# SuperbTUM/real-time-ReID-tracking

Hardware: AMD Instinct MI355X
Metric: crops/sec embedded + NxM distmat ms, ResNet18-SE 128x256 (higher is better)
Workload: dtype f16x3; 1 GPU; BASELINE configs[1]: ResNet18-SE embed 4096 distinct uint8 crops (128x256) per GPU + 4096x4096 L2 distmat; crops_per_gpu=4096, embed_dim=512, chunk=1024

## Files before the change

real-time-reid-tracking_amd/csrc/api.hip:

```cpp
#include "reid_internal.h"
#include <stdarg.h>
#include <stdio.h>
#include <string.h>
#include <stdlib.h>
#include <sstream>

static thread_local char g_err[1024] = "";

void reid_set_error(const char* fmt, ...) {
    va_list ap;
    va_start(ap, fmt);
    vsnprintf(g_err, sizeof(g_err), fmt, ap);
    va_end(ap);
}

extern "C" const char* reid_last_error(void) { return g_err; }

extern "C" int reid_device_count(int* n) {
    ARG_CHECK(n);
    HIP_TRY(hipGetDeviceCount(n));
    return REID_OK;
}

extern "C" int reid_ctx_create(int device, reid_ctx** out) {
// ... 7 lines not shown
    DeviceGuard _dev_guard(device);
    reid_ctx* c = new reid_ctx();
    c->device = device;
    if (const char* e = getenv("REID_SWIN_CHUNK_MAX")) {
        const int v = atoi(e);
        if (v > 0 && v < c->swin_chunk_cap) c->swin_chunk_cap = v;
    }
    if (const char* e = getenv("REID_KNN_WIDE_MIN")) c->knn_wide_min = atoll(e);
    HIP_TRY(hipStreamCreateWithFlags(&c->own_stream, hipStreamNonBlocking));
    c->stream = c->own_stream;
    HIP_TRY(hipHostMalloc((void**)&c->fault, 64, hipHostMallocMapped));
    memset(c->fault, 0, 64);
    HIP_TRY(hipEventCreate(&c->t0));
    HIP_TRY(hipEventCreate(&c->t1));
    *out = c;
    return REID_OK;
}

extern "C" int reid_ctx_destroy(reid_ctx* ctx) {
    if (!ctx) return REID_OK;
    DeviceGuard _dev_guard(ctx->device);
    hipStreamSynchronize(ctx->stream);
    comm_release(ctx);
    swin_release(ctx);
    for (int i = 0; i < 2; ++i)
        if (ctx->frame_ev[i]) hipEventDestroy(ctx->frame_ev[i]);
    if (ctx->copy_ev) hipEventDestroy(ctx->copy_ev);
    for (hipEvent_t e : ctx->pipe_ev) hipEventDestroy(e);
    for (int i = 0; i < 2; ++i) {
        if (ctx->fwd_ev[i]) hipEventDestroy(ctx->fwd_ev[i]);
        if (ctx->match_ev[i]) hipEventDestroy(ctx->match_ev[i]);
    }
    if (ctx->join_ev) hipEventDestroy(ctx->join_ev);
    if (ctx->match_stream) { hipStreamSynchronize(ctx->match_stream); hipStreamDestroy(ctx->match_stream); }
    if (ctx->copy_stream) { hipStreamSynchronize(ctx->copy_stream); hipStreamDestroy(ctx->copy_stream); }
    for (auto& kv : ctx->ws) hipFree(kv.second.first);
    for (auto& kv : ctx->split_w) hipFree(kv.second);
    for (auto& kv : ctx->pinned) hipHostFree(kv.second.first);
    if (ctx->se18.blob) hipFree(ctx->se18.blob);
    if (ctx->se18.blob16) hipFree(ctx->se18.blob16);
    if (ctx->se18.stem_w16) hipFree(ctx->se18.stem_w16);
    if (ctx->se18.stem_w16s) hipFree(ctx->se18.stem_w16s);
    for (int i = 0; i < 2; ++i)
        if (ctx->se18.l1_conv2_w16s[i]) hipFree(ctx->se18.l1_conv2_w16s[i]);
    if (ctx->se18.zero_page) hipFree(ctx->se18.zero_page);
    if (ctx->se18.ep) hipFree(ctx->se18.ep);
    for (auto& e : ctx->ev_pool) { hipEventDestroy(e.first); hipEventDestroy(e.second); }
    for (auto& p : ctx->pending) { hipEventDestroy(p.a); hipEventDestroy(p.b); }
    hipEventDestroy(ctx->t0);
    hipEventDestroy(ctx->t1);
    hipStreamDestroy(ctx->own_stream);
    if (ctx->fault) hipHostFree(ctx->fault);
    delete ctx;
    return REID_OK;
}

extern "C" int reid_ctx_set_stream(reid_ctx* ctx, void* s) {
    ARG_CHECK(ctx);
    CTX_GUARD(ctx);
    ctx->stream = s ? (hipStream_t)s : ctx->own_stream;
    return REID_OK;
}

extern "C" int reid_ctx_set_null_stream(reid_ctx* ctx) {
    ARG_CHECK(ctx);
    CTX_GUARD(ctx);
// ... 105 lines not shown
        reid_set_error("%s: side indices are pending (reid_ctx_set_side_index) but the loaded weights carry no table for them", what);
        ctx->side_idx.clear();
        return REID_ERR_STATE;
    }
    if (ctx->side_cursor + (size_t)n > ctx->side_idx.size()) {
        reid_set_error("%s: %d images but only %zu side indices are pending", what, n, ctx->side_idx.size() - ctx->side_cursor);
        ctx->side_idx.clear();
        return REID_ERR_ARG;
    }
    const int32_t* h = ctx->side_idx.data() + ctx->side_cursor;
    for (int i = 0; i < n; ++i)
        if (h[i] >= rows) {
            reid_set_error("%s: side index %d of image %d is outside the table of %d rows", what, h[i], i, rows);
            ctx->side_idx.clear();
            return REID_ERR_ARG;
        }
    int32_t* d;
    REID_TRY(ctx_ws(ctx, "side.idx", (size_t)n * 4, (void**)&d));
    HIP_TRY(hipMemcpyAsync(d, h, (size_t)n * 4, hipMemcpyHostToDevice, ctx->stream));
    HIP_TRY(hipStreamSynchronize(ctx->stream));
    ctx->side_cursor += n;
    if (ctx->side_cursor == ctx->side_idx.size()) ctx->side_idx.clear();
    *d_idx = d;
    return REID_OK;
}

extern "C" int reid_ctx_set_debug_keep(reid_ctx* ctx, int on) {
    ARG_CHECK(ctx);
    CTX_GUARD(ctx);
    ctx->debug_keep = on < 0 ? 0 : (on > 2 ? 2 : on);
    return REID_OK;
}

int ctx_ws(reid_ctx* ctx, const char* name, size_t bytes, void** out) {
    auto it = ctx->ws.find(name);
    if (it != ctx->ws.end() && it->second.second >= bytes) {
        *out = it->second.first;
        return REID_OK;
    }
    bool regrow = false;
    if (it != ctx->ws.end()) {
        HIP_TRY(hipStreamSynchronize(ctx->stream));
        HIP_TRY(hipFree(it->second.first));
        ctx->ws.erase(it);
        regrow = true;
    }
    void* p = nullptr;
    size_t cap = bytes < 256 ? 256 : bytes;
    if (regrow) cap += cap / 2 < ((size_t)1 << 30) ? cap / 2 : ((size_t)1 << 30);
    hipError_t e = hipMalloc(&p, cap);
    if (e != hipSuccess) {
        reid_set_error("hipMalloc(%zu) for workspace '%s' failed: %s", cap, name, hipGetErrorString(e));
        return REID_ERR_NOMEM;
    }
    ctx->ws[name] = {p, cap};
    *out = p;
    return REID_OK;
}

int ctx_pinned(reid_ctx* ctx, const char* name, size_t bytes, void** out) {
    auto it = ctx->pinned.find(name);
    if (it != ctx->pinned.end() && it->second.second >= bytes) {
        *out = it->second.first;
        return REID_OK;
    }
    if (it != ctx->pinned.end()) {
        HIP_TRY(hipStreamSynchronize(ctx->stream));
// ... 596 lines not shown
        REID_TRY(launch_norm_finalize(ctx, b.stats, n, tiles, k.c, half, hw, k.in_gamma, k.in_beta, k.bn1_scale, k.bn1_shift,
                                      b.a_scale, b.a_shift));
        REID_TRY(conv_gemm(ctx, A_IM2COL, c1, n, Ho, Wo, k.c, k.conv2_w, k.c, 3, 3, 1, 1, 9 * k.c, b.a_scale, b.a_shift, 1,
                           k.bn2_scale, k.bn2_shift, k.ds ? nullptr : cur, k.ds ? 0 : 1, b.stats, y));
        }
        const float* shortcut = cur;
        if (k.ds) {
            REID_TRY(conv_gemm(ctx, A_IM2COL, cur, n, H, W, k.cin, k.ds_w, k.c, 1, 1, k.stride, 0, k.cin, nullptr, nullptr, 0,
                               k.ds_scale, k.ds_shift, nullptr, 0, nullptr, sc, 0, cur16));
            shortcut = sc;
        }
        float* out = c1;
        if (w.arch == 1) {
            REID_TRY(launch_ta_tail(ctx, y, shortcut, n, Ho, Wo, k.c, k.ta, out));
        } else if (w.arch == 2) {
            REID_TRY(launch_ema_tail(ctx, y, shortcut, n, Ho, Wo, k.c, k.ema, out));
        } else if (ctx->f32_conv == 1) {
            bool fp32_read = true;
            if (cur16 && !keep && i < 7 && w.blk[i + 1].ds && ctx->pack_epilogue) {
                const Se18Block& nx = w.blk[i + 1];
                fp32_read = !(conv_split_path(ctx, n, Ho, Wo, nx.cin, nx.c, 3, 3, nx.stride, 1) &&
                              conv_split_path(ctx, n, Ho, Wo, nx.cin, nx.c, 1, 1, nx.stride, 0));
            }
            REID_TRY(launch_se_tail(ctx, b.stats, n, tiles, k.c, k.mid, hw, k.se_w1, k.se_w2, y, shortcut, fp32_read ? out : nullptr,
                                    i < 7 ? cur16 : nullptr));
        } else {
            REID_TRY(launch_se_finalize(ctx, b.stats, n, tiles, k.c, k.mid, hw, k.se_w1, k.se_w2, b.se));
            REID_TRY(launch_se_combine(ctx, y, shortcut, b.se, n, hw, k.c, out));
        }
        b.stage[2 + i] = out;
        cur = out;
        H = Ho;
        W = Wo;
    }
    REID_TRY(launch_gem_neck(ctx, cur, n, H * W, 512, w.gem_p, w.neck_scale, w.neck_shift, b.gem, d_emb));
    {
        const int32_t* d_cam;
        REID_TRY(ctx_take_side(ctx, n, w.num_cams, "reid_embed (camera bias)", &d_cam));
        if (d_cam) REID_TRY(launch_add_indexed_rows(ctx, d_emb, n, 1, 512, w.cam_bias, d_cam, w.cam_factor));
    }
    b.stage[10] = b.gem;
    if (d_logits) {
        if (!w.cls_w) {
            reid_set_error("logits requested but the weight blob has no classifier (cls.w)");
            return REID_ERR_STATE;
        }
        GemmParams p;
        memset(&p, 0, sizeof(p));
        p.A = d_emb; p.lda = 512;
        p.B = w.cls_w; p.ldb = 512;
        p.M = n; p.N = w.num_class; p.K = 512;
        p.C = d_logits; p.ldc = w.num_class;
        REID_TRY(launch_gemm_f32(ctx, A_DENSE, E_BIAS, p, REID_K_CONV_GEMM, 2.0 * n * w.num_class * 512,
                                 ((double)n * 512 + (double)w.num_class * 512 + (double)n * w.num_class) * 4.0));
    }
    ctx->last_n = n;
    ctx->last_f16 = false;
    for (int s = 0; s < 11; ++s) ctx->stage_ptr[s] = b.stage[s];
    return REID_OK;
}

int conv_gemm16(reid_ctx* ctx, int amode, const _Float16* x, int n, int H, int W, int Cin, const _Float16* wgt, int Cout,
                       int R, int S, int stride, int pad, int K, const float* col_scale, const float* col_shift,
                       const _Float16* residual, int relu, float* stats, _Float16* out, int Hp, int Wp) {
    Gemm16Params p;
    memset(&p, 0, sizeof(p));
// ... 160 lines not shown

extern "C" int reid_debug_stage(reid_ctx* ctx, int stage, float* out, size_t max_floats, size_t* count) {
    ARG_CHECK(ctx && stage >= 0 && stage < 11 && out);
    CTX_GUARD(ctx);
    if (!ctx->debug_keep || ctx->last_n <= 0) {
        reid_set_error("reid_debug_stage: enable reid_ctx_set_debug_keep before the embed call");
        return REID_ERR_STATE;
    }
    const size_t total = kStageElems[stage] * (size_t)ctx->last_n;
    if (count) *count = total;
    const size_t ncopy = total < max_floats ? total : max_floats;
    if (ctx->last_f16 && stage < 10) {
        std::vector<_Float16> tmp(ncopy);
        HIP_TRY(hipMemcpyAsync(tmp.data(), ctx->stage_ptr[stage], ncopy * 2, hipMemcpyDeviceToHost, ctx->stream));
        HIP_TRY(hipStreamSynchronize(ctx->stream));
        for (size_t i = 0; i < ncopy; ++i) out[i] = (float)tmp[i];
        return REID_OK;
    }
    HIP_TRY(hipMemcpyAsync(out, ctx->stage_ptr[stage], ncopy * 4, hipMemcpyDeviceToHost, ctx->stream));
    HIP_TRY(hipStreamSynchronize(ctx->stream));
    return REID_OK;
}

int ctx_pipe_events(reid_ctx* ctx, int passes) {
    if (!ctx->copy_stream) HIP_TRY(hipStreamCreateWithFlags(&ctx->copy_stream, hipStreamNonBlocking));
    while ((int)ctx->pipe_ev.size() < 2 * passes) {
        hipEvent_t e;
        HIP_TRY(hipEventCreateWithFlags(&e, hipEventDisableTiming));
        ctx->pipe_ev.push_back(e);
    }
    return REID_OK;
}

extern "C" int reid_embed_u8_dev(reid_ctx* ctx, const uint8_t* d_crops, int n, float* d_emb, float* d_logits) {
    ARG_CHECK(ctx && d_crops && d_emb && n >= 0);
    CTX_ENTER(ctx);
    const int nc = ctx->se18.num_class;
    for (int i = 0; i < n; i += ctx->chunk) {
        const int m = n - i < ctx->chunk ? n - i : ctx->chunk;
        REID_TRY(seres18_run(ctx, d_crops + (size_t)i * IMG_H * IMG_W * 3, true, m, d_emb + (size_t)i * 512,
                                 d_logits ? d_logits + (size_t)i * nc : nullptr));
    }
    return REID_OK;
}

extern "C" int reid_embed_u8(reid_ctx* ctx, const uint8_t* crops, int n, float* emb, float* logits) {
    ARG_CHECK(ctx && crops && emb && n >= 0);
    CTX_ENTER(ctx);
    if (n == 0) return REID_OK;
    const int nc = ctx->se18.num_class;
    uint8_t* d_in;
    float *d_emb, *d_log = nullptr;
    const size_t crop_b = (size_t)IMG_H * IMG_W * 3;
    REID_TRY(ctx_ws(ctx, "io.in", (size_t)n * crop_b, (void**)&d_in));
    REID_TRY(ctx_ws(ctx, "io.emb", (size_t)n * 512 * 4, (void**)&d_emb));
    if (logits) REID_TRY(ctx_ws(ctx, "io.logits", (size_t)n * nc * 4 + 16, (void**)&d_log));
    REID_TRY(host_passes(
        ctx, n, ctx->chunk,
        [&](int i, int m, hipStream_t s) -> int {
            HIP_TRY(hipMemcpyAsync(d_in + (size_t)i * crop_b, crops + (size_t)i * crop_b, (size_t)m * crop_b, hipMemcpyHostToDevice, s));
            return REID_OK;
        },
        [&](int i, int m) -> int {
            return seres18_run(ctx, d_in + (size_t)i * crop_b, true, m, d_emb + (size_t)i * 512, d_log ? d_log + (size_t)i * nc : nullptr);
        },
        [&](int i, int m, hipStream_t s) -> int {
            HIP_TRY(hipMemcpyAsync(emb + (size_t)i * 512, d_emb + (size_t)i * 512, (size_t)m * 512 * 4, hipMemcpyDeviceToHost, s));
            if (logits) HIP_TRY(hipMemcpyAsync(logits + (size_t)i * nc, d_log + (size_t)i * nc, (size_t)m * nc * 4, hipMemcpyDeviceToHost, s));
            return REID_OK;
        }));
    return ctx_fault_status(ctx);
}

extern "C" int reid_embed_f32_nchw_dev(reid_ctx* ctx, const float* d_x, int n, float* d_emb, float* d_logits) {
    ARG_CHECK(ctx && d_x && d_emb && n >= 0);
    CTX_ENTER(ctx);
    const int nc = ctx->se18.num_class;
    const size_t img = (size_t)IMG_H * IMG_W * 3;
    for (int i = 0; i < n; i += ctx->chunk) {
        const int m = n - i < ctx->chunk ? n - i : ctx->chunk;
        float* nhwc;
        REID_TRY(ctx_ws(ctx, "se18.in_nhwc", (size_t)m * img * 4, (void**)&nhwc));
        REID_TRY(launch_nchw_to_nhwc3(ctx, d_x + (size_t)i * img, m, IMG_H, IMG_W, nhwc));
        REID_TRY(seres18_run(ctx, nhwc, false, m, d_emb + (size_t)i * 512, d_logits ? d_logits + (size_t)i * nc : nullptr));
    }
    return REID_OK;
}

extern "C" int reid_embed_f32_nchw(reid_ctx* ctx, const float* x, int n, float* emb, float* logits) {
    ARG_CHECK(ctx && x && emb && n >= 0);
    CTX_ENTER(ctx);
    if (n == 0) return REID_OK;
    const int nc = ctx->se18.num_class;
    const size_t img = (size_t)IMG_H * IMG_W * 3;
    float *d_in, *d_emb, *d_log = nullptr;
    REID_TRY(ctx_ws(ctx, "io.in", (size_t)n * img * 4, (void**)&d_in));
    REID_TRY(ctx_ws(ctx, "io.emb", (size_t)n * 512 * 4, (void**)&d_emb));
    if (logits) REID_TRY(ctx_ws(ctx, "io.logits", (size_t)n * nc * 4 + 16, (void**)&d_log));
    REID_TRY(host_passes(
        ctx, n, ctx->chunk,
        [&](int i, int m, hipStream_t s) -> int {
            HIP_TRY(hipMemcpyAsync(d_in + (size_t)i * img, x + (size_t)i * img, (size_t)m * img * 4, hipMemcpyHostToDevice, s));
            return REID_OK;
        },
        [&](int i, int m) -> int {
            float* nhwc;
            REID_TRY(ctx_ws(ctx, "se18.in_nhwc", (size_t)m * img * 4, (void**)&nhwc));
            REID_TRY(launch_nchw_to_nhwc3(ctx, d_in + (size_t)i * img, m, IMG_H, IMG_W, nhwc));
            return seres18_run(ctx, nhwc, false, m, d_emb + (size_t)i * 512, d_log ? d_log + (size_t)i * nc : nullptr);
        },
        [&](int i, int m, hipStream_t s) -> int {
            HIP_TRY(hipMemcpyAsync(emb + (size_t)i * 512, d_emb + (size_t)i * 512, (size_t)m * 512 * 4, hipMemcpyDeviceToHost, s));
            if (logits) HIP_TRY(hipMemcpyAsync(logits + (size_t)i * nc, d_log + (size_t)i * nc, (size_t)m * nc * 4, hipMemcpyDeviceToHost, s));
            return REID_OK;
        }));
    return ctx_fault_status(ctx);
}

int embed_ragged_enqueue(reid_ctx* ctx, const char* tag, const uint8_t* packed, const int64_t* offsets, const int32_t* hw, int n,
// ... 519 lines not shown
```

real-time-reid-tracking_amd/csrc/conv3x3_f16.hip:

```cpp
#include "reid_internal.h"
#include "conv3x3_geom.h"
#include <type_traits>

typedef _Float16 f16;
typedef f16 half8 __attribute__((ext_vector_type(8)));
typedef float f32x16 __attribute__((ext_vector_type(16)));

namespace {

#define GPTR(p) ((const __attribute__((address_space(1))) void*)(p))
#define LPTR(p) ((__attribute__((address_space(3))) void*)(uintptr_t)(p))
#define WAIT_VMCNT(n) asm volatile("s_waitcnt vmcnt(%0)" ::"n"(n) : "memory")
#define RAW_BARRIER() asm volatile("s_barrier" ::: "memory")

template <int TW, int IMGS, int BN, int LW, bool SPLIT = false, bool PAIR = false>
__global__ __launch_bounds__(LW ? 768 : 512) void conv3x3_f16_kernel(const Gemm16Params p) {
    static_assert(!PAIR || (SPLIT && LW == 1 && BN == 128), "PAIR: fp32-class build, loader waves, 128-wide tiles");
    constexpr int TH = 256 / (IMGS * TW);
    constexpr int WP = TW + 2, HP = TH + 2;
    constexpr int NPX = IMGS * HP * WP;
    constexpr int NPI = (NPX + 7) / 8;
    constexpr int HPW = (NPI + 7) / 8;
    constexpr int HALO_BYTES = NPI * 1024;
    constexpr int B_BYTES = BN * 128;
// ... 699 lines not shown
        for (int a = 0; a < TM; ++a)
#pragma unroll
            for (int e = 0; e < 16; ++e) tile[c_row_natural<TW, IMGS>(wm, a, e, lh) * BN + lcol] = (f16)acc[a][b][e];
    }
    ESTAMP(te3);
    __syncthreads();
    constexpr int C8 = BN / 8;
    for (int idx = tid; idx < 256 * C8; idx += NTHR) {
        const int row = idx / C8, c8 = idx - row * C8;
        if (row < m_valid) *(half8*)(Cb + (long long)row * ldc + c8 * 8) = *(const half8*)(tile + row * BN + c8 * 8);
    }
    if (LW && p.diag && lane == 0 && blockIdx.x < 64) {
        asm volatile("s_waitcnt vmcnt(0)" ::: "memory");
        ESTAMP(te4);
        if (wave == 0) {
            unsigned long long* d2 = p.diag + 64 * 8 * 4 + blockIdx.x * 8;
            d2[0] = te1 - t_loop_end; d2[1] = te2 - te1; d2[2] = te3 - te2; d2[3] = te4 - te3;
        }
    }
}

template <int TW, int IMGS, int LW, bool SPLIT = false>
int launch_geom(reid_ctx* ctx, const Gemm16Params& p0) {
    Gemm16Params p = p0;
    p.fault = ctx->fault;
    p.general_epi = !ctx->split_lean_epi;
    p.pair_early = ctx->split_pair == 2;
    p.loader_prio = ctx->f16_loader_prio == 2 || (ctx->f16_loader_prio == 1 && SPLIT);
    p.frag_ahead = ctx->f16_frag_ahead;
    const int nmt = (p.M + 255) / 256;
    const int threads = LW ? 768 : 512;
    const int nchunk = p.Cin / 64;
    auto splitk = [&](int tiles, int bn, int sk) -> int {
        if (sk > 1) {
            float* ws;
            int* cnt;
            bool fresh = ctx->ws.find("conv16.splitk_cnt") == ctx->ws.end();
            REID_TRY(ctx_ws(ctx, "conv16.splitk_ws", (size_t)tiles * sk * 256 * bn * sizeof(float), (void**)&ws));
            REID_TRY(ctx_ws(ctx, "conv16.splitk_cnt", 256 * sizeof(int), (void**)&cnt));
            if (fresh) HIP_TRY(hipMemsetAsync(cnt, 0, 256 * sizeof(int), ctx->stream));
            p.split_k = sk; p.splitk_ws = ws; p.splitk_cnt = cnt;
        }
        return REID_OK;
    };
    const int tiles128 = p.N % 128 == 0 ? nmt * (p.N / 128) : 0;
#ifdef REID_EXPERIMENTS
    constexpr bool CAN_PAIR = SPLIT && LW == 1;
#else
    constexpr bool CAN_PAIR = false;
#endif
    const bool pair = CAN_PAIR && ctx->split_pair && p.split_terms == 3;
    if (tiles128 > 128) {
        if constexpr (CAN_PAIR) {
            if (pair) hipLaunchKernelGGL((conv3x3_f16_kernel<TW, IMGS, 128, LW, SPLIT, true>), dim3(tiles128), dim3(threads), 0, ctx->stream, p);
        }
        if (!pair) hipLaunchKernelGGL((conv3x3_f16_kernel<TW, IMGS, 128, LW, SPLIT>), dim3(tiles128), dim3(threads), 0, ctx->stream, p);
    } else {
        const int tiles64 = nmt * (p.N / 64);
        int best_bn = 64, best_sk = 1;
        double best = 1e30;
        auto consider = [&](int bn, int tiles, int sk, double bias) {
            if (tiles <= 0 || nchunk % sk != 0 || (sk > 1 && (!ctx->f16_split_k || tiles * sk > 256))) return;
            const double cost = (double)((tiles * sk + 255) / 256) * (nchunk / sk) * 9 * (bn == 128 ? 1.3 : 0.65) + (sk > 1 ? 2.0 : 0.0) + bias;
            if (cost < best) { best = cost; best_bn = bn; best_sk = sk; }
        };
        if (ctx->f16_wide_splitk && nchunk >= 16 && tiles128 >= 48) consider(128, tiles128, 4, -0.003);
// ... 137 lines not shown
```

real-time-reid-tracking_amd/csrc/conv3x3_x3.hip:

```cpp
#include "reid_internal.h"
#include "conv3x3_geom.h"
#include "lin_math.h"
#include <type_traits>
#include <utility>

typedef _Float16 f16;
typedef f16 half8 __attribute__((ext_vector_type(8)));
typedef float f32x16 __attribute__((ext_vector_type(16)));

namespace {

#define GPTR(p) ((const __attribute__((address_space(1))) void*)(p))
#define LPTR(p) ((__attribute__((address_space(3))) void*)(uintptr_t)(p))
#define RAW_BARRIER() asm volatile("s_barrier" ::: "memory")
#define LDS_READ(dst, addr, off) asm volatile("ds_read_b128 %0, %1 offset:%2" : "=v"(dst) : "v"(addr), "n"(off))

template <int N>
__device__ __forceinline__ void lgkm_wait2(half8& x, half8& y) { asm volatile("s_waitcnt lgkmcnt(%2)" : "+v"(x), "+v"(y) : "n"(N)); }
template <int N>
__device__ __forceinline__ void lgkm_wait1(half8& x) { asm volatile("s_waitcnt lgkmcnt(%1)" : "+v"(x) : "n"(N)); }

__device__ __forceinline__ void wait_vm(int n) {
    switch (n) {
        case 0: asm volatile("s_waitcnt vmcnt(0)" ::: "memory"); break;
// ... 1675 lines not shown
    while (ctx->f16_split_k && tiles * sk * 2 <= slots && ncr % (sk * 2) == 0 && sk * 2 <= (wide ? 8 : 4)) sk *= 2;
    const int cap = ctx->x3_sk_cap > 0 ? ctx->x3_sk_cap : 4;
    return sk > cap ? cap : sk;
}

static bool x3_wide_tiles(const reid_ctx* ctx, const Gemm16Params& p) {
    if (p.N % 128 != 0 || (p.W == 16 && (ctx->x3_narrow & 1)) || (p.W == 8 && (ctx->x3_narrow & 2))) return false;
    if (p.W == 8 && p.N == 256 && !(ctx->x3_narrow & 4)) {
        const int nmt = (p.M + 255) / 256, ncr = p.Cin / 3 / 32;
        const int t128 = nmt * 2, t64 = nmt * 4;
        const int s128 = x3_split(ctx, t128, ncr, true);
        (void)t64;
        if (t128 * s128 < 256) return false;
    }
    if (p.W == 8 && p.N == 512 && ctx->x3_l4_narrow_nmt > 0) {
        const int nmt = (p.M + 255) / 256, ncr = p.Cin / 3 / 32;
        const int t128 = nmt * 4, s128 = x3_split(ctx, t128, ncr, true);
        if (s128 == 4 && t128 * s128 > 256 && nmt <= ctx->x3_l4_narrow_nmt) return false;
        if (s128 == 1 && t128 % 256 != 0 && t128 % 256 <= 128) return false;
        if (s128 == 2 && t128 > 128 && t128 * 4 <= 768) return false;
    }
    return true;
}

static int x3_slots(const Gemm16Params& p, bool wide) { return (!wide && p.W == 8 && p.N == 512 && (p.M + 255) / 256 > 32) ? 768 : 512; }

template <int TW, int IMGS>
int launch_x3m16(reid_ctx* ctx, const Gemm16Params& p0) {
    Gemm16Params p = p0;
    const int nmt = (p.M + 255) / 256;
    const bool wide = x3_wide_tiles(ctx, p);
    const int tiles = nmt * (wide ? p.N / 128 : p.N / 64);
    const int sk = x3_split(ctx, tiles, p.Cin / 3 / 32, wide, x3_slots(p, wide));
    if (sk > 1) {
        float* ws;
        int* cnt;
        const bool fresh = ctx->ws.find("x3.splitk_cnt") == ctx->ws.end();
        ARG_CHECK(tiles <= 512);
        REID_TRY(ctx_ws(ctx, "x3.splitk_ws", (size_t)tiles * sk * 256 * (wide ? 128 : 64) * sizeof(float), (void**)&ws));
        REID_TRY(ctx_ws(ctx, "x3.splitk_cnt", 1024 * sizeof(int), (void**)&cnt));
        if (fresh) HIP_TRY(hipMemsetAsync(cnt, 0, 1024 * sizeof(int), ctx->stream));
        p.split_k = sk; p.splitk_ws = ws; p.splitk_cnt = cnt;
    } else {
        p.split_k = 1;
    }
    const bool unrolled = ctx->x3_unroll && (long long)p.M * (p.Cin / 3) * 4 < 0x7f000000ll && (long long)p.N * p.ldb * 2 < 0x7f000000ll;
    if (wide && unrolled) hipLaunchKernelGGL((conv3x3_x3u_kernel<TW, IMGS, 128, 2>), dim3(tiles * sk), dim3(256), 0, ctx->stream, p);
    else if (wide) hipLaunchKernelGGL((conv3x3_x3m16_kernel<TW, IMGS, 128>), dim3(tiles * sk), dim3(256), 0, ctx->stream, p);
    else if (unrolled && ctx->x3_unroll == 3) hipLaunchKernelGGL((conv3x3_x3u_kernel<TW, IMGS, 64, 3>), dim3(tiles * sk), dim3(256), 0, ctx->stream, p);
#ifdef REID_EXPERIMENTS
    else if (unrolled && ctx->x3_unroll == 4) hipLaunchKernelGGL((conv3x3_x3u_kernel<TW, IMGS, 64, 4>), dim3(tiles * sk), dim3(256), 0, ctx->stream, p);
    else if (unrolled && ctx->x3_unroll == 5) hipLaunchKernelGGL((conv3x3_x3u_kernel<TW, IMGS, 64, 3, 3>), dim3(tiles * sk), dim3(256), 0, ctx->stream, p);
#endif
    else hipLaunchKernelGGL((conv3x3_x3m16_kernel<TW, IMGS, 64>), dim3(tiles * sk), dim3(256), 0, ctx->stream, p);
    return REID_OK;
}

template <int TW, int IMGS>
void launch_x3(reid_ctx* ctx, const Gemm16Params& p) {
    const int nmt = (p.M + 255) / 256;
    if (p.N % 128 == 0) hipLaunchKernelGGL((conv3x3_x3_kernel<TW, IMGS, 128>), dim3(nmt * (p.N / 128)), dim3(256), 0, ctx->stream, p);
    else hipLaunchKernelGGL((conv3x3_x3_kernel<TW, IMGS, 64>), dim3(nmt * (p.N / 64)), dim3(256), 0, ctx->stream, p);
}

}

static int launch_tiles(const reid_ctx* ctx, const Gemm16Params& p) {
    const int nmt = (p.M + 255) / 256;
    return nmt * (x3_wide_tiles(ctx, p) ? p.N / 128 : p.N / 64);
}

bool conv3x3_x3_supported(const reid_ctx* ctx, const Gemm16Params& p) {
    if (!ctx->split_x3 || p.split_terms != 3 || p.Cin % 96 != 0 || p.N % 64 != 0 || p.M % 128 != 0 || !conv3x3_f16_supported(p)) return false;
    if (p.relu_from % 16 != 0 || (p.pack16 && p.pack_from % 32 != 0)) return false;
    if (p.N % 128 != 0 && ctx->split_x3 < 3) return false;
    const int nmt = (p.M + 255) / 256;
    const long long blocks = (long long)nmt * (p.N % 128 == 0 ? p.N / 128 : p.N / 64);
    if (blocks >= ctx->split_x3_min_blocks) return true;
    if (ctx->split_x3 < 2 || !ctx->split_x3_small) return false;
    if (ctx->split_x3_small == 1) return true;
    const int tiles = launch_tiles(ctx, p);
    if (p.W == 8) return true;
    if (p.W == 32) return p.M / 256 > 256 || tiles >= 384;
    return p.M / 256 > 128 || tiles >= 384;
}

int launch_conv3x3_x3(reid_ctx* ctx, const Gemm16Params& p0) {
    Gemm16Params p = p0;
    p.fault = ctx->fault;
    p.ablate |= ctx->x3_ablate;
    if (ctx->split_x3 >= 2) {
        if (p.W == 32) REID_TRY((launch_x3m16<32, 1>(ctx, p)));
        else if (p.W == 16) REID_TRY((launch_x3m16<16, 1>(ctx, p)));
        else REID_TRY((launch_x3m16<8, 2>(ctx, p)));
    } else if (p.W == 32) launch_x3<32, 1>(ctx, p);
    else if (p.W == 16) launch_x3<16, 1>(ctx, p);
    else launch_x3<8, 2>(ctx, p);
    LAUNCH_CHECK();
    return REID_OK;
}

#ifdef REID_EXPERIMENTS
int launch_chain(reid_ctx* ctx, const ChainParams& cp, int W) {
    ARG_CHECK(cp.n_img >= 1 && cp.n_img <= 64 && cp.n_stages >= 1 && cp.n_stages <= 8 && cp.counters && W == 8);
    const int blocks = cp.total_items < 512 ? cp.total_items : 512;
    hipLaunchKernelGGL((chain_kernel<8, 2, 128>), dim3(blocks), dim3(256), 0, ctx->stream, cp);
    LAUNCH_CHECK();
    return REID_OK;
}
#endif

bool conv_x3s_supported(const reid_ctx* ctx, const Gemm16Params& p) {
    if (!ctx->conv_x3s || ctx->split_x3 < 2 || p.split_terms != 3 || p.Cin % 96 != 0 || p.N % 128 != 0 || p.M % 128 != 0) return false;
    if (!((p.R == 1 || p.R == 3) && p.S == p.R && p.pad == (p.R - 1) / 2 && (p.stride == 1 || p.stride == 2))) return false;
    if (p.R == 3 && p.stride == 1) return false;
    if (p.relu_from % 16 != 0 || (p.pack16 && p.pack_from % 32 != 0)) return false;
    const long long a_bytes = (long long)(p.M / (p.Ho * p.Wo)) * p.H * p.W * (p.Cin / 3) * 4;
    return a_bytes < 0x7f000000ll && 128ll * p.ldb * 2 < 0x7f000000ll && 256ll * p.ldc * 4 < 0x7f000000ll && (long long)p.M * 2 < 0x7f000000ll;
}

int launch_conv_x3s(reid_ctx* ctx, const Gemm16Params& p0, int kind, double flops, double bytes) {
    Gemm16Params p = p0;
    p.fault = ctx->fault;
    p.ablate = 0;
    const int tiles = ((p.M + 255) / 256) * (p.N / 128), nq = p.R * p.S * (p.Cin / 3 / 32);
    int sk = 1;
    while (ctx->f16_split_k && tiles * sk * 2 <= 512 && nq / (sk * 2) >= 2 && sk * 2 <= ctx->x3s_sk_cap) sk *= 2;
    if (sk > 1) {
        float* ws;
        int* cnt;
        const bool fresh = ctx->ws.find("x3.splitk_cnt") == ctx->ws.end();
        ARG_CHECK(tiles <= 512);
        REID_TRY(ctx_ws(ctx, "x3.splitk_ws", (size_t)tiles * sk * 256 * 128 * sizeof(float), (void**)&ws));
        REID_TRY(ctx_ws(ctx, "x3.splitk_cnt", 1024 * sizeof(int), (void**)&cnt));
        if (fresh) HIP_TRY(hipMemsetAsync(cnt, 0, 1024 * sizeof(int), ctx->stream));
        p.split_k = sk; p.splitk_ws = ws; p.splitk_cnt = cnt;
    } else {
        p.split_k = 1;
    }
    prof_begin(ctx, kind, flops, bytes);
    hipLaunchKernelGGL((conv_x3s_kernel<128>), dim3(tiles * sk), dim3(256), 0, ctx->stream, p);
    prof_end(ctx);
    LAUNCH_CHECK();
    return REID_OK;
}

bool lin_x3_supported(const reid_ctx* ctx, const Gemm16Params& p) {
    const int Kr = p.K / 3;
    return ctx->lin_x3 && ctx->split_x3 >= 2 && p.lin && p.split_terms == 3 && p.K % 96 == 0 && p.N % 128 == 0 && p.n_real == p.N && p.lda == 2 * Kr &&
           p.ldb == 3 * Kr && !p.scat_h && !p.par4 && (p.C32 != nullptr) != (p.pack_out != 0) &&
           256ll * p.lda * 2 < 0x7f000000ll && 128ll * p.ldb * 2 < 0x7f000000ll && 256ll * p.ldc * 4 < 0x7f000000ll;
}

int launch_lin_x3(reid_ctx* ctx, const Gemm16Params& p0, int kind, double flops, double bytes) {
    Gemm16Params p = p0;
    p.fault = ctx->fault;
    p.ablate = ctx->x3_ablate;
    p.stats = nullptr; p.col_scale = nullptr; p.relu = 0; p.split_k = 1;
    if (p.pack_out) {
        p.pack16 = p.C;
// ... 12 lines not shown
```

real-time-reid-tracking_amd/csrc/debug.hip:

```cpp
#include "reid_internal.h"
#include <string.h>
#include <stdlib.h>
#include <vector>

namespace {
struct Switch { const char* name; int reid_ctx::* field; };
const Switch kSwitches[] = {
    {"f16_cfg", &reid_ctx::f16_cfg}, {"f16_lin_256", &reid_ctx::f16_lin_256}, {"f16_split_k", &reid_ctx::f16_split_k},
    {"bank_fast", &reid_ctx::bank_fast}, {"side_copy", &reid_ctx::side_copy}, {"f32_stem_pool", &reid_ctx::f32_stem_pool},
    {"stem_split", &reid_ctx::stem_split}, {"split_pair", &reid_ctx::split_pair}, {"split_lean_epi", &reid_ctx::split_lean_epi},
    {"knn_wide", &reid_ctx::knn_wide}, {"f16_loader_prio", &reid_ctx::f16_loader_prio}, {"f16_frag_ahead", &reid_ctx::f16_frag_ahead},
    {"pack_epilogue", &reid_ctx::pack_epilogue}, {"f16_wide_splitk", &reid_ctx::f16_wide_splitk}, {"f32_split_k", &reid_ctx::f32_split_k},
    {"swin_fold", &reid_ctx::swin_fold}, {"swin_stop", &reid_ctx::swin_stop}, {"select_two_pass", &reid_ctx::select_two_pass},
    {"split_terms", &reid_ctx::split_terms}, {"f32_conv", &reid_ctx::f32_conv}, {"swin_attn_mfma", &reid_ctx::swin_attn_mfma},
    {"swin_attn_split", &reid_ctx::swin_attn_split}, {"swin_two_linear", &reid_ctx::swin_two_linear},
    {"f16_loader_waves", &reid_ctx::f16_loader_waves}, {"f16_halo", &reid_ctx::f16_halo}, {"f16_stem_fused", &reid_ctx::f16_stem_fused},
    {"f16_se_tail", &reid_ctx::f16_se_tail}, {"f16_c64", &reid_ctx::f16_c64}, {"swin_chunk_cap", &reid_ctx::swin_chunk_cap},
    {"split_x3", &reid_ctx::split_x3}, {"x3_ablate", &reid_ctx::x3_ablate}, {"x3_unroll", &reid_ctx::x3_unroll}, {"x3_narrow", &reid_ctx::x3_narrow}, {"conv_x3s", &reid_ctx::conv_x3s}, {"x3s_sk_cap", &reid_ctx::x3s_sk_cap}, {"x3_l4_narrow_nmt", &reid_ctx::x3_l4_narrow_nmt}, {"split_x3_small", &reid_ctx::split_x3_small}, {"split_x3_min_blocks", &reid_ctx::split_x3_min_blocks}, {"f32_dist_bk16", &reid_ctx::f32_dist_bk16}, {"lin_x3", &reid_ctx::lin_x3},
    {"host_pipeline", &reid_ctx::host_pipeline}, {"x3_sk_cap", &reid_ctx::x3_sk_cap}, {"chain", &reid_ctx::chain}, {"split_gemm_min_tiles", &reid_ctx::split_gemm_min_tiles},
    {"rerank_hbm_acc", &reid_ctx::rerank_hbm_acc},
};
}

extern "C" int reid_debug_set_switch(reid_ctx* ctx, const char* name, long long value) {
    ARG_CHECK(ctx && name);
    CTX_GUARD(ctx);
    HIP_TRY(hipStreamSynchronize(ctx->stream));
    if (!strcmp(name, "knn_wide_min")) {
        ctx->knn_wide_min = value;
        return REID_OK;
    }
    for (const Switch& s : kSwitches)
        if (!strcmp(name, s.name)) {
            if (!strcmp(name, "split_terms") && value != 3 && value != 4) break;
            ctx->*(s.field) = (int)value;
            return REID_OK;
        }
    reid_set_error("reid_debug_set_switch: no switch '%s' (or a value it does not take)", name);
    return REID_ERR_ARG;
}

extern "C" int reid_debug_get_switch(reid_ctx* ctx, const char* name, long long* value) {
    ARG_CHECK(ctx && name && value);
    if (!strcmp(name, "knn_wide_min")) {
        *value = ctx->knn_wide_min;
        return REID_OK;
    }
    for (const Switch& s : kSwitches)
        if (!strcmp(name, s.name)) {
            *value = ctx->*(s.field);
            return REID_OK;
        }
    reid_set_error("reid_debug_get_switch: no switch '%s'", name);
// ... 770 lines not shown
```

real-time-reid-tracking_amd/csrc/elementwise.hip:

```cpp
#include "reid_internal.h"
#include <math.h>

typedef float f32x4 __attribute__((ext_vector_type(4)));

namespace {

__device__ __forceinline__ float wave_sum(float v) {
#pragma unroll
    for (int o = 32; o > 0; o >>= 1) v += __shfl_xor(v, o);
    return v;
}
__device__ __forceinline__ double wave_sum_d(double v) {
#pragma unroll
    for (int o = 32; o > 0; o >>= 1) v += __shfl_xor(v, o);
    return v;
}

__global__ void nchw_to_nhwc3_kernel(const float* __restrict__ x, long long npix, int hw, float* __restrict__ out) {
    for (long long i = blockIdx.x * (long long)blockDim.x + threadIdx.x; i < npix; i += (long long)gridDim.x * blockDim.x) {
        const long long img = i / hw;
        const int p = (int)(i - img * hw);
        const float* src = x + img * 3 * hw + p;
        float* dst = out + i * 3;
        dst[0] = src[0];
// ... 201 lines not shown
        if (lane == 0) hid[m] = fmaxf(acc, 0.f);
    }
    __syncthreads();
    for (int ch = tid; ch < c; ch += 256) {
        float acc = 0.f;
        for (int m = 0; m < mid; ++m) acc += w2[m * c + ch] * hid[m];
        s[(long long)img * c + ch] = 1.0f / (1.0f + expf(-acc));
    }
}

__global__ void se_combine_kernel(const float* __restrict__ y, const float* __restrict__ sc, const float* __restrict__ s,
                                  long long total4, int hw, int c, float* __restrict__ out) {
    const int c4n = c >> 2;
    for (long long i = blockIdx.x * (long long)blockDim.x + threadIdx.x; i < total4; i += (long long)gridDim.x * blockDim.x) {
        const int cc = (int)(i % c4n);
        const long long pix = i / c4n;
        const long long img = pix / hw;
        const f32x4 yy = *(const f32x4*)(y + i * 4);
        const f32x4 rr = *(const f32x4*)(sc + i * 4);
        const f32x4 ss = *(const f32x4*)(s + img * c + cc * 4);
        f32x4 o = ss * yy + rr;
        o.x = fmaxf(o.x, 0.f); o.y = fmaxf(o.y, 0.f); o.z = fmaxf(o.z, 0.f); o.w = fmaxf(o.w, 0.f);
        *(f32x4*)(out + i * 4) = o;
    }
}

template <bool SMALL>
__global__ __launch_bounds__(256) void se_tail_kernel(const float* __restrict__ stats, int tiles, int c, int mid, int hw,
                                                      const float* __restrict__ w1, const float* __restrict__ w2,
                                                      const float* __restrict__ y, const float* __restrict__ sc, int rows,
                                                      float* __restrict__ out, _Float16* __restrict__ packed, int* __restrict__ fault) {
    __shared__ __attribute__((aligned(16))) float pooled[512];
    __shared__ float hid[64];
    __shared__ __attribute__((aligned(16))) float gate[512];
    const int img = blockIdx.y, tid = threadIdx.x, lane = tid & 63, wave = tid >> 6;
    constexpr int MJ = SMALL ? 8 : 16, MW2 = 32;
    f32x4 w1v[SMALL ? 8 : 1][2];
    float w2v[SMALL ? 2 : 1][SMALL ? MW2 : 1];
    if constexpr (SMALL) {
        const int c4v = c >> 2;
#pragma unroll
        for (int j = 0; j < MJ; ++j)
#pragma unroll
            for (int k = 0; k < 2; ++k) {
                const int m = wave + 4 * j, c4 = lane + 64 * k;
                if (m < mid && c4 < c4v) w1v[j][k] = *(const f32x4*)(w1 + (long long)m * c + c4 * 4);
            }
#pragma unroll
        for (int q = 0; q < 2; ++q)
#pragma unroll
            for (int m = 0; m < MW2; ++m) {
                const int ch = tid + 256 * q;
                if (ch < c && m < mid) w2v[q][m] = w2[m * c + ch];
            }
    }
    for (int ch = tid; ch < c; ch += 256) {
        double acc = 0.0;
        for (int t = 0; t < tiles; ++t) acc += (double)stats[(((long long)img * tiles + t) * c + ch) * 2];
        pooled[ch] = (float)(acc / hw);
    }
    __syncthreads();
    {
        const int c4v = c >> 2;
        float acc[16];
#pragma unroll
        for (int j = 0; j < 16; ++j) {
            acc[j] = 0.f;
// ... 295 lines not shown
```

real-time-reid-tracking_amd/csrc/reid_internal.h:

```cpp
#pragma once
#include <hip/hip_runtime.h>
#include <stdint.h>
#include <stddef.h>
#include <stdio.h>
#include <string>
#include <map>
#include <tuple>
#include <vector>
#include "../../include/reid_hip.h"
struct reid_ctx;

void reid_set_error(const char* fmt, ...);

#define HIP_TRY(expr)                                                                         \
    do {                                                                                      \
        hipError_t _e = (expr);                                                               \
        if (_e != hipSuccess) {                                                               \
            reid_set_error("%s:%d %s -> %s", __FILE__, __LINE__, #expr, hipGetErrorString(_e)); \
            return REID_ERR_HIP;                                                              \
        }                                                                                     \
    } while (0)

#define REID_TRY(expr)            \
    do {                          \
// ... 118 lines not shown
    int* fault;
};

__device__ __forceinline__ float l2sqr_of(float dot, float rs, float cq) { return fmaf(-2.0f, dot, rs + cq); }

__device__ __forceinline__ unsigned range_acc(unsigned m, float v) {
    const unsigned b = __float_as_uint(v) & 0x7fffffffu;
    return b > m ? b : m;
}
__device__ __forceinline__ void range_raise(int* fault, unsigned m) {
    if (fault && m >= 0x477fe000u) fault[0] = 1;
}

template <class P>
inline void set_scatter(P& p, int scat_h, int scat_w, int py, int px) {
    p.scat_h = scat_h; p.scat_w = scat_w; p.scat_py = py; p.scat_px = px;
    p.scat_mhw = p.scat_mw = 0;
    if (scat_h > 0) {
        p.scat_mhw = (unsigned)(((1ull << 32) + (unsigned long long)(scat_h * scat_w) - 1) / (unsigned long long)(scat_h * scat_w));
        p.scat_mw = (unsigned)(((1ull << 32) + (unsigned long long)scat_w - 1) / (unsigned long long)scat_w);
    }
}

struct reid_ctx;
int launch_gemm_f16(reid_ctx* ctx, int amode, const Gemm16Params& p, int kind, double flops, double bytes);
bool conv3x3_f16_supported(const Gemm16Params& p);
int launch_conv3x3_f16(reid_ctx* ctx, const Gemm16Params& p, int kind, double flops, double bytes);
int launch_conv3x3_split(reid_ctx* ctx, const Gemm16Params& p, int kind, double flops, double bytes);
bool conv3x3_x3_supported(const reid_ctx* ctx, const Gemm16Params& p);
int launch_conv3x3_x3(reid_ctx* ctx, const Gemm16Params& p);
bool lin_x3_supported(const reid_ctx* ctx, const Gemm16Params& p);
int launch_lin_x3(reid_ctx* ctx, const Gemm16Params& p, int kind, double flops, double bytes);
bool conv_x3s_supported(const reid_ctx* ctx, const Gemm16Params& p);
int launch_conv_x3s(reid_ctx* ctx, const Gemm16Params& p, int kind, double flops, double bytes);
int launch_gemm_f16_split(reid_ctx* ctx, const Gemm16Params& p, int kind, double flops, double bytes);
bool two_linear_supported(const reid_ctx*, long long T, int C, int hid);
int launch_two_linear(reid_ctx*, const _Float16* a16, long long T, int C, int hid, const float* w1, const float* b1, const float* w2,
                      const float* b2, int act, const float* res, float* out, const float* x32 = nullptr, const float* ln_g = nullptr,
                      const float* ln_b = nullptr);
bool ln_linear_supported(const reid_ctx*, long long T, int C, int n);
int launch_ln_linear(reid_ctx*, const float* x32, const float* ln_g, const float* ln_b, long long T, int C, int n, const float* w, const float* bias,
                     float* out, int ldc);
int launch_window_attn_cos(reid_ctx* ctx, int mode, const void* qkv, int ldq, int n_img, int H, int W, int heads, int shifted,
                           const float* bias_t, const float* scale, void* out);
int launch_post_norm(reid_ctx* ctx, int side_mode, const float* x, const float* y, long long T, int C, const float* g, const float* b,
                     float* out, _Float16* side);
int launch_split_pack(reid_ctx* ctx, const float* x, long long rows, int C, _Float16* out, const float* d_scale = nullptr);
int launch_split_weights(reid_ctx* ctx, const float* w, int cout, int taps, int cin, int terms, _Float16* out, const float* d_scale = nullptr);
int launch_prep_u8_pad_f16(reid_ctx*, const uint8_t* crops, int n, int h, int w, int hp, int wp, _Float16* out);
int launch_prep_f32_pad_f16(reid_ctx*, const float* nhwc3, int n, int h, int w, int hp, int wp, _Float16* out);
int launch_maxpool3s2_f16(reid_ctx*, const _Float16* x, int n, int h, int w, int c, _Float16* out);
int launch_affine_relu_f16(reid_ctx*, _Float16* x, const float* a_scale, const float* a_shift, int n_img, int hw, int c);
int launch_norm_apply_f16(reid_ctx*, _Float16* x, const float* stats, int n_img, int tiles, int c, int half, int hw,
                          const float* in_gamma, const float* in_beta, const float* bn_scale, const float* bn_shift);
int launch_se_tail_f16(reid_ctx*, const float* stats, int n_img, int tiles, int c, int mid, int hw, const float* w1, const float* w2t,
                       const _Float16* y, const _Float16* sc, _Float16* out);
int launch_se_combine_f16(reid_ctx*, const _Float16* y, const _Float16* sc, const float* s, int n_img, int hw, int c,
                          _Float16* out);
int launch_gem_neck_f16(reid_ctx*, const _Float16* x, int n_img, int hw, int c, const float* p, const float* scale,
                        const float* shift, float* gem_out, float* emb);
int launch_f32_to_f16(reid_ctx*, const float* x, size_t n, _Float16* out);
int launch_stem_w16(reid_ctx*, const float* stem_w_f32, _Float16* out);
bool conv3x3_c64_f16_supported(int H, int W, int Cin, int Cout, int R, int S, int stride, int pad);
int launch_scale_rows_f16(reid_ctx*, const float* w, const float* scale, int rows, int k, _Float16* out);
int launch_conv3x3_c64_f16(reid_ctx*, const _Float16* in, int n, const _Float16* w_scaled, const float* shift,
                           const _Float16* residual, int relu, float* stats, _Float16* out, const _Float16* zero_page,
// ... 152 lines not shown
    int select_two_pass = 0;
    int rerank_hbm_acc = 0;
    int swin_stop = -1;
    int swin_fold = 1;
    int swin_two_linear = 1;
    int swin_attn_split = 0;
    int two_linear_ablate = 0;
    int swin_attn_mfma = 1;
    int f16_split_k = 1;
    int swin_chunk_cap = 1024;
    int f16_lin_256 = 1;
    int f16_cfg = 0;
    int frame_m[2] = {0, 0};
    float* frame_emb[2] = {nullptr, nullptr};
    int frame_pending[2] = {0, 0}, frame_has[2] = {0, 0};
    size_t frame_tm[2] = {0, 0};
    hipEvent_t frame_ev[2] = {nullptr, nullptr};
    hipStream_t match_stream = nullptr;
    int match_async = 0;
    hipEvent_t join_ev = nullptr;
    hipEvent_t fwd_ev[2] = {nullptr, nullptr}, match_ev[2] = {nullptr, nullptr};
    hipStream_t copy_stream = nullptr;
    hipEvent_t copy_ev = nullptr;
    std::vector<hipEvent_t> pipe_ev;
    int host_pipeline = 1;
    int side_copy = 1;
    std::vector<int32_t> side_idx;
    size_t side_cursor = 0;
    const char* frame_out[2] = {nullptr, nullptr};
    float* stage_ptr[11] = {nullptr};
    unsigned long long* conv_diag = nullptr;
    std::string split_bad_se18, split_bad_swin;
    int* fault = nullptr;
};
enum { REID_FAULT_RANGE = 1, REID_FAULT_NONFINITE = 2 };
int ctx_fault_status(reid_ctx* ctx);
bool knn_wide_eligible(reid_ctx* ctx, int nq, int nb, int d, int k);
int knn_wide_dev(reid_ctx* ctx, const float* xp, int nq, const float* yp, int nb, int ld, const float* rs, const float* cq, int k, float* d_D,
                 int32_t* d_I);

inline std::string split_range_violation(const float* blob, const std::map<std::string, std::pair<size_t, size_t>>& tab,
                                         const std::vector<std::pair<std::string, float>>& suffix_bound) {
    for (const auto& kv : tab) {
        for (const auto& sb : suffix_bound) {
            const std::string& suf = sb.first;
            if (kv.first.size() < suf.size() || kv.first.compare(kv.first.size() - suf.size(), suf.size(), suf) != 0) continue;
            float mx = 0.f;
            const float* w = blob + kv.second.first;
            for (size_t i = 0; i < kv.second.second; ++i) {
                const float a = w[i] < 0 ? -w[i] : w[i];
                if (!(a <= mx)) mx = a;
            }
            if (!(mx < sb.second)) {
                char buf[160];
                snprintf(buf, sizeof(buf), "%s (max |w| = %g, limit %g)", kv.first.c_str(), (double)mx, (double)sb.second);
                return buf;
            }
            break;
        }
    }
    return std::string();
}

struct ChainElem {
    const float* x;
    const float* stats;
    const float* sc;
    const float *g, *b;
// ... 118 lines not shown
```

Before: 85160 crops/s.

## Run embedding chunk passes on two staggered streams to overlap ResNet passes

Adds a second 'lane' stream so consecutive chunk passes of the SE-ResNet18 embedding alternate between the main stream and a lane stream. Each pass waits on the previous pass's mid-network event, so the tail of one chunk overlaps the head of the next. Workspaces are namespaced per lane. Lanes are enabled only when no split-K rendezvous kernels would be launched, which guards against a deadlock when two passes share the GPU. It also aliases the SE gate buffer onto the pooled shared-memory array to cut LDS use. The cost is twice the workspace memory and added event synchronisation.

```diff
diff --git a/real-time-reid-tracking_amd/csrc/api.hip b/real-time-reid-tracking_amd/csrc/api.hip
--- a/real-time-reid-tracking_amd/csrc/api.hip
+++ b/real-time-reid-tracking_amd/csrc/api.hip
@@ -63,6 +63,12 @@
         if (ctx->match_ev[i]) hipEventDestroy(ctx->match_ev[i]);
     }
     if (ctx->join_ev) hipEventDestroy(ctx->join_ev);
+    if (ctx->lane_fork_ev) hipEventDestroy(ctx->lane_fork_ev);
+    for (int i = 0; i < 2; ++i) {
+        if (ctx->lane_mid_ev[i]) hipEventDestroy(ctx->lane_mid_ev[i]);
+        if (ctx->lane_end_ev[i]) hipEventDestroy(ctx->lane_end_ev[i]);
+    }
+    if (ctx->lane_stream) { hipStreamSynchronize(ctx->lane_stream); hipStreamDestroy(ctx->lane_stream); }
     if (ctx->match_stream) { hipStreamSynchronize(ctx->match_stream); hipStreamDestroy(ctx->match_stream); }
     if (ctx->copy_stream) { hipStreamSynchronize(ctx->copy_stream); hipStreamDestroy(ctx->copy_stream); }
     for (auto& kv : ctx->ws) hipFree(kv.second.first);
@@ -234,7 +240,9 @@
     return REID_OK;
 }
 
-int ctx_ws(reid_ctx* ctx, const char* name, size_t bytes, void** out) {
+int ctx_ws(reid_ctx* ctx, const char* name0, size_t bytes, void** out) {
+    const std::string lane_name = ctx->lane ? std::string("lane1.") + name0 : std::string();
+    const char* name = ctx->lane ? lane_name.c_str() : name0;
     auto it = ctx->ws.find(name);
     if (it != ctx->ws.end() && it->second.second >= bytes) {
         *out = it->second.first;
@@ -897,6 +905,10 @@
         cur = out;
         H = Ho;
         W = Wo;
+        if (ctx->lane_mid && i + 1 == ctx->embed_lanes_mid) {
+            HIP_TRY(hipEventRecord(ctx->lane_mid, ctx->stream));
+            ctx->lane_mid = nullptr;
+        }
     }
     REID_TRY(launch_gem_neck(ctx, cur, n, H * W, 512, w.gem_p, w.neck_scale, w.neck_shift, b.gem, d_emb));
     {
@@ -1123,16 +1135,127 @@
     return REID_OK;
 }
 
+
+static int conv_pass_split_k(reid_ctx* ctx, int n, int H, int W, int Cin, int Cout, int R, int stride, int pack_from) {
+    const int pad = (R - 1) / 2;
+    if (!conv_split_path(ctx, n, H, W, Cin, Cout, R, R, stride, pad)) return 0;
+    Gemm16Params q;
+    memset(&q, 0, sizeof(q));
+    const int T = ctx->split_terms;
+    q.split_terms = T;
+    q.H = H; q.W = W; q.Cin = T * Cin; q.R = R; q.S = R; q.stride = stride; q.pad = pad;
+    q.Ho = (H + 2 * pad - R) / stride + 1;
+    q.Wo = (W + 2 * pad - R) / stride + 1;
+    q.M = n * q.Ho * q.Wo; q.N = Cout; q.K = R * R * T * Cin; q.ldb = q.K; q.ldc = Cout;
+    q.relu_from = q.pack_from = pack_from;
+    if (R == 3 && stride == 1 && conv3x3_f16_supported(q)) {
+        if (conv3x3_x3_supported(ctx, q)) return conv3x3_x3_split_k(ctx, q);
+        return q.N % 128 == 0 && ((q.M + 255) / 256) * (q.N / 128) > 128 ? 1 : 0;
+    }
+    if (conv_x3s_supported(ctx, q)) return conv_x3s_split_k(ctx, q);
+    return 1;
+}
+
+static bool pass_lane_ok(reid_ctx* ctx, int n) {
+    const Se18Weights& w = ctx->se18;
+    if (ctx->precision != 2 || !w.loaded || w.arch != 0 || ctx->f32_conv != 1 || !w.zero_page || !ctx->pack_epilogue || ctx->chain) return false;
+    int H = 64, W = 32;
+    for (int i = 0; i < 8; ++i) {
+        const Se18Block& k = w.blk[i];
+        const int half = k.ibn ? k.c / 2 : 0;
+        if (conv_pass_split_k(ctx, n, H, W, k.cin, k.c, 3, k.stride, half) != 1) return false;
+        const int Ho = (H + 2 - 3) / k.stride + 1, Wo = (W + 2 - 3) / k.stride + 1;
+        if (conv_pass_split_k(ctx, n, Ho, Wo, k.c, k.c, 3, 1, 0) != 1) return false;
+        if (k.ds && conv_pass_split_k(ctx, n, H, W, k.cin, k.c, 1, k.stride, 0) != 1) return false;
+        H = Ho;
+        W = Wo;
+    }
+    return true;
+}
+
+static int lanes_create(reid_ctx* ctx) {
+    if (ctx->lane_stream) return REID_OK;
+    HIP_TRY(hipStreamCreateWithFlags(&ctx->lane_stream, hipStreamNonBlocking));
+    HIP_TRY(hipEventCreateWithFlags(&ctx->lane_fork_ev, hipEventDisableTiming));
+    for (int i = 0; i < 2; ++i) {
+        HIP_TRY(hipEventCreateWithFlags(&ctx->lane_mid_ev[i], hipEventDisableTiming));
+        HIP_TRY(hipEventCreateWithFlags(&ctx->lane_end_ev[i], hipEventDisableTiming));
+    }
+    return REID_OK;
+}
+
+template <class Run>
+static int embed_passes_dev(reid_ctx* ctx, int n, Run run) {
+    const int chunk = ctx->chunk;
+    ctx->embed_lanes_used = 0;
+    const bool lanes = n > chunk && ctx->embed_lanes >= 2 && !ctx->profile && !ctx->debug_keep && pass_lane_ok(ctx, chunk);
+    if (!lanes) {
+        for (int i = 0; i < n; i += chunk) REID_TRY(run(i, n - i < chunk ? n - i : chunk));
+        return REID_OK;
+    }
+    REID_TRY(lanes_create(ctx));
+    hipStream_t const main_stream = ctx->stream;
+    hipStream_t const st[2] = {main_stream, ctx->lane_stream};
+    bool busy1 = false, need_fork = true, prev_full = false;
+    int prev_lane = -1, rc = REID_OK;
+    auto hip = [&](hipError_t e, const char* what) {
+        if (e != hipSuccess && rc == REID_OK) {
+            reid_set_error("embed lanes: %s -> %s", what, hipGetErrorString(e));
+            rc = REID_ERR_HIP;
+        }
+    };
+    auto join = [&]() {
+        if (busy1) hip(hipStreamWaitEvent(main_stream, ctx->lane_end_ev[1], 0), "join");
+        busy1 = false;
+        prev_lane = -1;
+        need_fork = true;
+    };
+    int k = 0;
+    for (int i = 0; i < n && rc == REID_OK; i += chunk, ++k) {
+        const int m = n - i < chunk ? n - i : chunk;
+        if (m != chunk && !pass_lane_ok(ctx, m)) {
+            join();
+            if (rc == REID_OK) rc = run(i, m);
+            continue;
+        }
+        const int lane = k & 1;
+        if (need_fork) {
+            hip(hipEventRecord(ctx->lane_fork_ev, main_stream), "fork");
+            hip(hipStreamWaitEvent(st[1], ctx->lane_fork_ev, 0), "fork");
+            need_fork = false;
+        }
+        if (prev_lane >= 0 && prev_lane != lane)
+            hip(hipStreamWaitEvent(st[lane], prev_full ? ctx->lane_end_ev[prev_lane] : ctx->lane_mid_ev[prev_lane], 0), "stagger");
+        if (rc != REID_OK) break;
+        const size_t n_split = ctx->split_w.size();
+        ctx->stream = st[lane];
+        ctx->lane = lane;
+        ctx->lane_mode = true;
+        ctx->lane_mid = ctx->lane_mid_ev[lane];
+        rc = run(i, m);
+        ctx->lane_mode = false;
+        ctx->lane = 0;
+        ctx->stream = main_stream;
+        if (rc == REID_OK && ctx->lane_mid) hip(hipEventRecord(ctx->lane_mid, st[lane]), "stagger");
+        ctx->lane_mid = nullptr;
+        hip(hipEventRecord(ctx->lane_end_ev[lane], st[lane]), "end of pass");
+        prev_full = ctx->split_w.size() != n_split;
+        prev_lane = lane;
+        if (lane == 1) busy1 = true;
+        if (rc == REID_OK) ctx->embed_lanes_used += 1;
+    }
+    join();
+    return rc;
+}
+
 extern "C" int reid_embed_u8_dev(reid_ctx* ctx, const uint8_t* d_crops, int n, float* d_emb, float* d_logits) {
     ARG_CHECK(ctx && d_crops && d_emb && n >= 0);
     CTX_ENTER(ctx);
     const int nc = ctx->se18.num_class;
-    for (int i = 0; i < n; i += ctx->chunk) {
-        const int m = n - i < ctx->chunk ? n - i : ctx->chunk;
-        REID_TRY(seres18_run(ctx, d_crops + (size_t)i * IMG_H * IMG_W * 3, true, m, d_emb + (size_t)i * 512,
-                                 d_logits ? d_logits + (size_t)i * nc : nullptr));
-    }
-    return REID_OK;
+    return embed_passes_dev(ctx, n, [&](int i, int m) -> int {
+        return seres18_run(ctx, d_crops + (size_t)i * IMG_H * IMG_W * 3, true, m, d_emb + (size_t)i * 512,
+                           d_logits ? d_logits + (size_t)i * nc : nullptr);
+    });
 }
 
 extern "C" int reid_embed_u8(reid_ctx* ctx, const uint8_t* crops, int n, float* emb, float* logits) {
@@ -1168,14 +1291,12 @@
     CTX_ENTER(ctx);
     const int nc = ctx->se18.num_class;
     const size_t img = (size_t)IMG_H * IMG_W * 3;
-    for (int i = 0; i < n; i += ctx->chunk) {
-        const int m = n - i < ctx->chunk ? n - i : ctx->chunk;
+    return embed_passes_dev(ctx, n, [&](int i, int m) -> int {
         float* nhwc;
         REID_TRY(ctx_ws(ctx, "se18.in_nhwc", (size_t)m * img * 4, (void**)&nhwc));
         REID_TRY(launch_nchw_to_nhwc3(ctx, d_x + (size_t)i * img, m, IMG_H, IMG_W, nhwc));
-        REID_TRY(seres18_run(ctx, nhwc, false, m, d_emb + (size_t)i * 512, d_logits ? d_logits + (size_t)i * nc : nullptr));
-    }
-    return REID_OK;
+        return seres18_run(ctx, nhwc, false, m, d_emb + (size_t)i * 512, d_logits ? d_logits + (size_t)i * nc : nullptr);
+    });
 }
 
 extern "C" int reid_embed_f32_nchw(reid_ctx* ctx, const float* x, int n, float* emb, float* logits) {
diff --git a/real-time-reid-tracking_amd/csrc/conv3x3_f16.hip b/real-time-reid-tracking_amd/csrc/conv3x3_f16.hip
--- a/real-time-reid-tracking_amd/csrc/conv3x3_f16.hip
+++ b/real-time-reid-tracking_amd/csrc/conv3x3_f16.hip
@@ -755,6 +755,7 @@
     const int threads = LW ? 768 : 512;
     const int nchunk = p.Cin / 64;
     auto splitk = [&](int tiles, int bn, int sk) -> int {
+        REID_TRY(lane_rendezvous_check(ctx, sk, "conv3x3_f16"));
         if (sk > 1) {
             float* ws;
             int* cnt;
diff --git a/real-time-reid-tracking_amd/csrc/conv3x3_x3.hip b/real-time-reid-tracking_amd/csrc/conv3x3_x3.hip
--- a/real-time-reid-tracking_amd/csrc/conv3x3_x3.hip
+++ b/real-time-reid-tracking_amd/csrc/conv3x3_x3.hip
@@ -1731,6 +1731,7 @@
     const bool wide = x3_wide_tiles(ctx, p);
     const int tiles = nmt * (wide ? p.N / 128 : p.N / 64);
     const int sk = x3_split(ctx, tiles, p.Cin / 3 / 32, wide, x3_slots(p, wide));
+    REID_TRY(lane_rendezvous_check(ctx, sk, "conv3x3_x3"));
     if (sk > 1) {
         float* ws;
         int* cnt;
@@ -1767,6 +1768,12 @@
 static int launch_tiles(const reid_ctx* ctx, const Gemm16Params& p) {
     const int nmt = (p.M + 255) / 256;
     return nmt * (x3_wide_tiles(ctx, p) ? p.N / 128 : p.N / 64);
+}
+
+int conv3x3_x3_split_k(const reid_ctx* ctx, const Gemm16Params& p) {
+    if (ctx->split_x3 < 2) return 1;
+    const bool wide = x3_wide_tiles(ctx, p);
+    return x3_split(ctx, launch_tiles(ctx, p), p.Cin / 3 / 32, wide, x3_slots(p, wide));
 }
 
 bool conv3x3_x3_supported(const reid_ctx* ctx, const Gemm16Params& p) {
@@ -1818,13 +1825,21 @@
     return a_bytes < 0x7f000000ll && 128ll * p.ldb * 2 < 0x7f000000ll && 256ll * p.ldc * 4 < 0x7f000000ll && (long long)p.M * 2 < 0x7f000000ll;
 }
 
+static int x3s_split(const reid_ctx* ctx, const Gemm16Params& p) {
+    const int tiles = ((p.M + 255) / 256) * (p.N / 128), nq = p.R * p.S * (p.Cin / 3 / 32);
+    int sk = 1;
+    while (ctx->f16_split_k && tiles * sk * 2 <= 512 && nq / (sk * 2) >= 2 && sk * 2 <= ctx->x3s_sk_cap) sk *= 2;
+    return sk;
+}
+int conv_x3s_split_k(const reid_ctx* ctx, const Gemm16Params& p) { return x3s_split(ctx, p); }
+
 int launch_conv_x3s(reid_ctx* ctx, const Gemm16Params& p0, int kind, double flops, double bytes) {
     Gemm16Params p = p0;
     p.fault = ctx->fault;
     p.ablate = 0;
-    const int tiles = ((p.M + 255) / 256) * (p.N / 128), nq = p.R * p.S * (p.Cin / 3 / 32);
-    int sk = 1;
-    while (ctx->f16_split_k && tiles * sk * 2 <= 512 && nq / (sk * 2) >= 2 && sk * 2 <= ctx->x3s_sk_cap) sk *= 2;
+    const int tiles = ((p.M + 255) / 256) * (p.N / 128);
+    const int sk = x3s_split(ctx, p);
+    REID_TRY(lane_rendezvous_check(ctx, sk, "conv_x3s"));
     if (sk > 1) {
         float* ws;
         int* cnt;
diff --git a/real-time-reid-tracking_amd/csrc/debug.hip b/real-time-reid-tracking_amd/csrc/debug.hip
--- a/real-time-reid-tracking_amd/csrc/debug.hip
+++ b/real-time-reid-tracking_amd/csrc/debug.hip
@@ -19,6 +19,7 @@
     {"split_x3", &reid_ctx::split_x3}, {"x3_ablate", &reid_ctx::x3_ablate}, {"x3_unroll", &reid_ctx::x3_unroll}, {"x3_narrow", &reid_ctx::x3_narrow}, {"conv_x3s", &reid_ctx::conv_x3s}, {"x3s_sk_cap", &reid_ctx::x3s_sk_cap}, {"x3_l4_narrow_nmt", &reid_ctx::x3_l4_narrow_nmt}, {"split_x3_small", &reid_ctx::split_x3_small}, {"split_x3_min_blocks", &reid_ctx::split_x3_min_blocks}, {"f32_dist_bk16", &reid_ctx::f32_dist_bk16}, {"lin_x3", &reid_ctx::lin_x3},
     {"host_pipeline", &reid_ctx::host_pipeline}, {"x3_sk_cap", &reid_ctx::x3_sk_cap}, {"chain", &reid_ctx::chain}, {"split_gemm_min_tiles", &reid_ctx::split_gemm_min_tiles},
     {"rerank_hbm_acc", &reid_ctx::rerank_hbm_acc},
+    {"embed_lanes", &reid_ctx::embed_lanes}, {"embed_lanes_mid", &reid_ctx::embed_lanes_mid}, {"embed_lanes_used", &reid_ctx::embed_lanes_used},
 };
 }
 
diff --git a/real-time-reid-tracking_amd/csrc/elementwise.hip b/real-time-reid-tracking_amd/csrc/elementwise.hip
--- a/real-time-reid-tracking_amd/csrc/elementwise.hip
+++ b/real-time-reid-tracking_amd/csrc/elementwise.hip
@@ -257,7 +257,7 @@
                                                       float* __restrict__ out, _Float16* __restrict__ packed, int* __restrict__ fault) {
     __shared__ __attribute__((aligned(16))) float pooled[512];
     __shared__ float hid[64];
-    __shared__ __attribute__((aligned(16))) float gate[512];
+    float* const gate = pooled;
     const int img = blockIdx.y, tid = threadIdx.x, lane = tid & 63, wave = tid >> 6;
     constexpr int MJ = SMALL ? 8 : 16, MW2 = 32;
     f32x4 w1v[SMALL ? 8 : 1][2];
diff --git a/real-time-reid-tracking_amd/csrc/reid_internal.h b/real-time-reid-tracking_amd/csrc/reid_internal.h
--- a/real-time-reid-tracking_amd/csrc/reid_internal.h
+++ b/real-time-reid-tracking_amd/csrc/reid_internal.h
@@ -174,6 +174,8 @@
 bool lin_x3_supported(const reid_ctx* ctx, const Gemm16Params& p);
 int launch_lin_x3(reid_ctx* ctx, const Gemm16Params& p, int kind, double flops, double bytes);
 bool conv_x3s_supported(const reid_ctx* ctx, const Gemm16Params& p);
+int conv3x3_x3_split_k(const reid_ctx* ctx, const Gemm16Params& p);
+int conv_x3s_split_k(const reid_ctx* ctx, const Gemm16Params& p);
 int launch_conv_x3s(reid_ctx* ctx, const Gemm16Params& p, int kind, double flops, double bytes);
 int launch_gemm_f16_split(reid_ctx* ctx, const Gemm16Params& p, int kind, double flops, double bytes);
 bool two_linear_supported(const reid_ctx*, long long T, int C, int hid);
@@ -392,8 +394,23 @@
     unsigned long long* conv_diag = nullptr;
     std::string split_bad_se18, split_bad_swin;
     int* fault = nullptr;
+    int embed_lanes = 2;
+    int embed_lanes_mid = 4;
+    int embed_lanes_used = 0;
+    int lane = 0;
+    bool lane_mode = false;
+    hipStream_t lane_stream = nullptr;
+    hipEvent_t lane_fork_ev = nullptr, lane_mid_ev[2] = {nullptr, nullptr}, lane_end_ev[2] = {nullptr, nullptr};
+    hipEvent_t lane_mid = nullptr;
 };
 enum { REID_FAULT_RANGE = 1, REID_FAULT_NONFINITE = 2 };
+inline int lane_rendezvous_check(const reid_ctx* ctx, int sk, const char* who) {
+    if (sk > 1 && ctx->lane_mode) {
+        reid_set_error("%s: a split-K launch (%d blocks per tile wait for each other) was reached while two pass lanes are in flight", who, sk);
+        return REID_ERR_STATE;
+    }
+    return REID_OK;
+}
 int ctx_fault_status(reid_ctx* ctx);
 bool knn_wide_eligible(reid_ctx* ctx, int nq, int nb, int d, int k);
 int knn_wide_dev(reid_ctx* ctx, const float* xp, int nq, const float* yp, int nb, int ld, const float* rs, const float* cq, int k, float* d_D,
```

Result: slower. 81490 crops/s (-4.3%).
